# ClashLuke/LocAtE

Hardware: AMD Instinct MI355X
Metric: images/sec (G+D step) 64x64 bs=64 (higher is better)
Workload: dtype f32 (contractions fp32-faithful on the matrix cores: 2 x scaled fp16 operand pieces / 3 MFMAs per slice where the operand's largest magnitude comes with it, else 3 x bf16 pieces / 6 MFMAs; fp32 accumulate); 1 GPU; LocAtE G+D step, 64x64 RGB, batch 64 per GPU (the fp32 variant - the reference's own precision - of BASELINE.json configs[1]: 64x64 RGB bs 64), self/feature attention at 16x16 and 64x64, random-init weights; global_batch=64, image_size=64, parallelism=dp1, launch=hipGraph replay, G-step generator pass on a second stream

## Files before the change

locate_amd/csrc/conv.hip:

```cpp
#include "igemm.h"

template <int WGM, int WGN, int TM, int TN>
__global__ void __launch_bounds__(256) conv_igemm_kernel(const IgParams p) {
    constexpr int BK = IG_BK;
    constexpr int BM = WGM * TM * 32;
    constexpr int BN = WGN * TN * 32;
    constexpr int KPT = BK * BN / 256;
    constexpr int A_F4 = BK * BM / 4;
    constexpr int A_PT = (A_F4 + 255) / 256;
    static_assert(WGM * WGN == 4, "four waves");
    static_assert(BN % 64 == 0 && KPT == 8, "one 8-row group of the offset table per thread and step");
    static_assert(BK <= IG_TAIL, "panel tail shorter than the prefetch distance (one stage beyond the last)");

    __shared__ __attribute__((aligned(16))) float As[2][BK][BM];
    __shared__ __attribute__((aligned(16))) float Bs[2][BK][BN];

    int bx, by, bz;
    xcd_tile(bx, by, bz, p.tile_nphase);
    const int zphase = bz / p.ksplit, zsplit = bz - zphase * p.ksplit;
    const IgPhase& ph = p.ph[zphase];
    const int N = p.B * ph.QH * ph.QW;
    const int n0 = bx * BN;
    const int m0 = by * BM;
    if (n0 >= N) return;
// ... 91 lines not shown
        }
        __builtin_amdgcn_sched_barrier(0);
        store_tiles(buf ^ 1);
        __syncthreads();
    }

    igemm_epilogue<WGM, WGN, TM, TN>(p, ph, acc, col_scale, N, n0, m0, zsplit, wm, wn, lane, nullptr, p.ksplit > 1);
}

#define B6_BK 16

#define IG_FOUR_BLOCKS_TILES 3
#define IG_FOUR_BLOCKS_MIN 2
template <int WGM, int WGN, int TM, int TN, int NP, int NW = 4>
__global__ void __launch_bounds__(64 * NW, (NW == 8 ? 1 : (WGM * TM > 4 ? 2 : ((WGM * TM * TN <= IG_FOUR_BLOCKS_TILES && WGM * TM * TN >= IG_FOUR_BLOCKS_MIN && NP <= 2) ? 4 : 3)))) conv_igemm_bx6_kernel(const IgParams p) {
    constexpr int BK = 4 * NW, KB = BK / 8, KS = BK / 16, NT = 64 * NW;
    constexpr int BM = WGM * TM * 32;
    constexpr int BN = WGN * TN * 32;
    static_assert(NW == 4 || NW == 8, "four or eight waves");
    static_assert(WGM * WGN == NW, "wave grid");
    static_assert(BN == 128 && KB * BN == NT, "one gathered fragment (k-block) per thread and stage");
    static_assert(KB * BM <= 2 * NT, "at most two weight fragments per thread and stage");
    static_assert(B6_BK == 16, "the host's split-K accounting counts 16-deep steps");
    constexpr bool A2 = KB * BM > NT;
    static_assert(2 * BK <= IG_TAIL && (IG_TAIL % 8) == 0, "panel tail shorter than the prefetch distance");

    constexpr int A_U4 = 2 * NP * KB * BM, B_U4 = 2 * NP * KB * BN;
    constexpr int EPI_U4 = (NW * 32 * 33 + 8 + 3) / 4;
    constexpr int SMEM_U4 = A_U4 + B_U4 > EPI_U4 ? A_U4 + B_U4 : EPI_U4;
    __shared__ uint4 smem[SMEM_U4];
    uint4 (*As)[NP][KB][BM] = reinterpret_cast<uint4 (*)[NP][KB][BM]>(smem);
    uint4 (*Bs)[NP][KB][BN] = reinterpret_cast<uint4 (*)[NP][KB][BN]>(smem + A_U4);

    int bx, by, bz;
    xcd_tile(bx, by, bz, p.tile_nphase);
    const int zphase = bz / p.ksplit, zsplit = bz - zphase * p.ksplit;
    const IgPhase& ph = p.ph[zphase];
    const int N = p.B * ph.QH * ph.QW;
    const int n0 = bx * BN;
    const int m0 = by * BM;
    if (n0 >= N) return;

    const int tid = threadIdx.x, lane = tid & 63, wid = tid >> 6;
// ... 91 lines not shown
            Bs[buf][NP - 1][kgrp][ncol] = l;
        } else {
            bf16x8 h;
#pragma unroll
            for (int j = 0; j < 8; ++j) h[j] = (__bf16)breg[j];
            Bs[buf][0][kgrp][ncol] = *reinterpret_cast<uint4*>(&h);
        }
    };

    if (nsteps > 0) {
        issue_loads();
        store_tiles(0);
        issue_loads();
    }
    __syncthreads();
    const int lrow = lane >> 5, lcol = lane & 31;
    constexpr int PROD = NP == 3 ? 6 : (NP == 2 ? 3 : 1);
    constexpr int NMF = TM * TN * PROD, HALF = KS == 1 ? NMF / 2 : NMF;
    using frag_t = typename std::conditional<NP == 2, f16x8, bf16x8>::type;
    for (int s = 0; s < nsteps; ++s) {
        const int buf = s & 1;
        frag_t a[TM][NP], b[TN][NP];
        auto fragments = [&](int ksub) {
#pragma unroll
            for (int i = 0; i < TM; ++i)
#pragma unroll
                for (int q = 0; q < NP; ++q) a[i][q] = *reinterpret_cast<const frag_t*>(&As[buf][q][2 * ksub + lrow][(wm * TM + i) * 32 + lcol]);
#pragma unroll
            for (int j = 0; j < TN; ++j)
#pragma unroll
// ... 32 lines not shown
            mfmas(HALF, NMF);
        } else {
            fragments(1);
            mfmas(0, NMF);
        }
        if constexpr (NP >= 2) {
#pragma unroll
            for (int k = 0; k < (KS == 1 ? NMF - HALF : NMF); ++k) {
                __builtin_amdgcn_sched_group_barrier(0x008, 1, 0);
                __builtin_amdgcn_sched_group_barrier(0x020, 1, 0);
                __builtin_amdgcn_sched_group_barrier(0x002, 3, 0);
            }
        }
        __syncthreads();
    }
    if constexpr (NP == 2) {
#pragma unroll
        for (int i = 0; i < TM; ++i)
#pragma unroll
            for (int j = 0; j < TN; ++j)
#pragma unroll
                for (int r = 0; r < 16; ++r) acc[i][j][r] = (acc[i][j][r] * a_unscale) * b_unscale;
    }
    float* const stage = reinterpret_cast<float*>(smem) + wid * (32 * 33);
    bool combined = false;
    if (p.ksplit > 1 && p.combine) {
        constexpr int FR = TM * TN * 4;
        const int tile = (zphase * (int)gridDim.y + by) * (int)gridDim.x + bx;
        const int ntiles = p.nphase * (int)gridDim.y * (int)gridDim.x;
        const unsigned tile_bytes = FR * NT * 16;
        __amdgpu_buffer_rsrc_t srs = __builtin_amdgcn_make_buffer_rsrc(p.slab, 0, (int)((unsigned)p.ksplit * ntiles * tile_bytes), 0x00020000);
        const unsigned my = ((unsigned)(zsplit * ntiles + tile)) * tile_bytes + (unsigned)tid * 16u;
#pragma unroll
        for (int i = 0; i < TM; ++i)
#pragma unroll
            for (int j = 0; j < TN; ++j)
#pragma unroll
                for (int q = 0; q < 4; ++q) {
                    u32x4 v;
                    v[0] = __float_as_uint(acc[i][j][4 * q + 0]); v[1] = __float_as_uint(acc[i][j][4 * q + 1]);
                    v[2] = __float_as_uint(acc[i][j][4 * q + 2]); v[3] = __float_as_uint(acc[i][j][4 * q + 3]);
                    __builtin_amdgcn_raw_buffer_store_b128(v, srs, (int)(my + (unsigned)(((i * TN + j) * 4 + q) * NT * 16)), 0, 16);
                }
        asm volatile("s_waitcnt vmcnt(0)" ::: "memory");
        __syncthreads();
        unsigned* const flag = reinterpret_cast<unsigned*>(smem) + NW * 32 * 33 + 4;
        if (tid == 0) {
            const unsigned ticket = __hip_atomic_fetch_add(p.counters + tile, 1u, __ATOMIC_RELAXED, __HIP_MEMORY_SCOPE_AGENT);
            const bool last = ticket == (unsigned)(p.ksplit - 1);
            if (last) {
                __hip_atomic_store(p.counters + tile, 0u, __ATOMIC_RELAXED, __HIP_MEMORY_SCOPE_AGENT);
                __builtin_amdgcn_fence(__ATOMIC_ACQUIRE, "agent");
                asm volatile("s_waitcnt vmcnt(0)" ::: "memory");
            }
            *flag = last ? 1u : 0u;
        }
        __syncthreads();
        if (*flag == 0u) return;
        const unsigned t0 = (unsigned)tile * tile_bytes + (unsigned)tid * 16u;
        const unsigned zstride = (unsigned)ntiles * tile_bytes;
#pragma unroll
// ... 14 lines not shown
                        v[zz][f] = __builtin_amdgcn_raw_buffer_load_b128(srs, (int)(t0 + (unsigned)(z0 + zz) * zstride + (unsigned)((h0 + f) * NT * 16)), 0, 16);
#pragma unroll
                for (int zz = 0; zz < ZB; ++zz)
#pragma unroll
                    for (int f = 0; f < HB; ++f) {
                        const int g = h0 + f, i = g / (TN * 4), j = (g / 4) % TN, q = g % 4;
#pragma unroll
                        for (int e = 0; e < 4; ++e) acc[i][j][4 * q + e] += __uint_as_float(v[zz][f][e]);
                    }
            }
        }
        __syncthreads();
        combined = true;
    }
    igemm_epilogue<WGM, WGN, TM, TN>(p, ph, acc, col_scale, N, n0, m0, combined ? 0 : zsplit, wm, wn, lane, stage, p.ksplit > 1 && !combined);
}

__global__ void __launch_bounds__(256) igemm_slab_reduce_kernel(const float* __restrict__ slab, float* __restrict__ out,
                                                                const float* __restrict__ bias, const float* __restrict__ scale,
                                                                int scale_bg, int scale_stride, int B, int M, int plane,
                                                                long long out_bs, long long slab_stride, int ksplit,
                                                                float* __restrict__ act_out, long long act_bs,
                                                                const float* __restrict__ mul_pre, long long mul_bs,
                                                                unsigned* __restrict__ out_absmax) {
    const unsigned per_b = (unsigned)M * (unsigned)plane;
    const unsigned total = (unsigned)B * per_b;
    const unsigned stride = gridDim.x * blockDim.x;
    const DivU32 dpb(per_b), dpl((unsigned)plane);
    float am = 0.0f;
    for (unsigned i = blockIdx.x * blockDim.x + threadIdx.x; i < total; i += stride) {
// ... 280 lines not shown
                                                                              p.out_bs, p.slab_stride, p.ksplit, p.act_out, p.act_bs, p.mul_pre, p.mul_bs, p.out_absmax);
}

template <int NP>
static void launch_bx6(const IgParams& p, dim3 grid, int bm, bool w8, hipStream_t st) {
    if (w8) {
        if (bm == 128) conv_igemm_bx6_kernel<2, 4, 2, 1, NP, 8><<<grid, 512, 0, st>>>(p);
        else conv_igemm_bx6_kernel<2, 4, 1, 1, NP, 8><<<grid, 512, 0, st>>>(p);
        return;
    }
    with_tile<true>(bm, [&](auto t) { using T = decltype(t); conv_igemm_bx6_kernel<T::wgm, T::wgn, T::tm, T::tn, NP><<<grid, 256, 0, st>>>(p); });
}

static int launch_igemm(IgParams& p, int nmax, void* slab_ws, unsigned* counters, hipStream_t st, const char* who) {
    p.tile_nphase = (path_disabled("phasefast") || (long long)p.OH * p.OW < 1024) ? 1 : p.nphase;
    if (p.win) return launch_win_igemm(p, nmax, slab_ws, counters, st, who);
    if (skinny_ok(p)) {
        p.ksplit = 1;
        launch_skinny(p, st);
        LOCATE_LAUNCH_CHECK(who);
        return LOCATE_OK;
    }
    if (pointwise_ok(p)) {
        p.ksplit = 1;
        launch_pointwise(p, st);
        LOCATE_LAUNCH_CHECK(who);
        return LOCATE_OK;
    }
    const int bm = igemm_bm(p.M, nmax, p.nphase);
    const SplitPlan sp = igemm_split_plan(p, nmax, counters != nullptr);
    p.ksplit = sp.ksplit;
    p.combine = sp.combine;
    p.counters = counters;
    p.slab = static_cast<float*>(slab_ws);
    p.slab_stride = (long long)p.B * p.M * p.OH * p.OW;
    dim3 grid(sp.gx, sp.gy, p.nphase * p.ksplit);
    for (int i = 0; i < p.nphase; ++i)
        LOCATE_REQUIRE(round_up(p.M, bm) <= p.ph[i].ld, "%s: tile height %d does not divide the panel width %d", who, bm, p.ph[i].ld);
    if (p.precision == 3) {
        launch_fp8_igemm(p, grid, bm, st);
        LOCATE_LAUNCH_CHECK(who);
        if (p.ksplit > 1 && !p.combine) {
            LOCATE_REQUIRE(p.slab_stride < (1ll << 31), "%s: split-K output of %lld elements exceeds the 32-bit index range", who, p.slab_stride);
            launch_slab_reduce(p, st);
            LOCATE_LAUNCH_CHECK(who);
        }
        return LOCATE_OK;
    }
    const bool w8 = !path_disabled("w8") && !path_disabled("bx6") && (bm == 128 || bm == 64) &&
                    (long long)grid.x * grid.y * grid.z <= knob_int("LOCATE_W8_MAX", 320);
// ... 405 lines not shown
                     static_cast<unsigned*>(counters), precision, static_cast<const unsigned*>(x_absmax), as_stream(stream), "locate_conv_fwd",
                     static_cast<const LocateActEpilogue*>(act_epilogue));
}

LOCATE_API int locate_conv_dgrad(const int* geom, const float* gy, int64_t gy_bs, const float* panel, const float* scale,
                                 int scale_group_batch, int scale_stride, const float* bias, float* gx, int64_t gx_bs,
                                 void* workspace, void* counters, int precision, const void* gy_absmax, const void* act_epilogue,
                                 void* stream) {
    const ConvGeom g = make_geom(geom);
    if (int e = geom_check(g, "locate_conv_dgrad")) return e;
    LOCATE_REQUIRE(gy && panel && gx, "locate_conv_dgrad: null pointer");
    return run_igemm(g, 1, gy, gy_bs, panel, scale, scale_group_batch, scale_stride, bias, gx, gx_bs,
                     static_cast<float*>(workspace), static_cast<unsigned*>(counters), precision, static_cast<const unsigned*>(gy_absmax),
                     as_stream(stream), "locate_conv_dgrad", static_cast<const LocateActEpilogue*>(act_epilogue));
}
```

locate_amd/csrc/convfp8.hip:

```cpp
#include "igemm.h"

__device__ __forceinline__ uint4 quant_fp8x16(const float (&v)[16], float sc) {
    unsigned w[4];
#pragma unroll
    for (int q = 0; q < 4; ++q) {
        int t = 0;
        t = __builtin_amdgcn_cvt_pk_fp8_f32(v[4 * q + 0] * sc, v[4 * q + 1] * sc, t, false);
        t = __builtin_amdgcn_cvt_pk_fp8_f32(v[4 * q + 2] * sc, v[4 * q + 3] * sc, t, true);
        w[q] = (unsigned)t;
    }
    return make_uint4(w[0], w[1], w[2], w[3]);
}

template <int WGM, int WGN, int TM, int TN>
__global__ void __launch_bounds__(256, (WGM * TM > 4 ? 2 : 3)) conv_igemm_fp8_kernel(const IgParams p) {
    constexpr int BK = 32, KB = 2, NT = 256, NW = 4;
    constexpr int BM = WGM * TM * 32;
    constexpr int BN = WGN * TN * 32;
    static_assert(WGM * WGN == NW && BN == 128 && KB * BN == NT, "one gathered chunk (16 k) per thread and stage");
    static_assert(KB * BM <= 2 * NT, "at most two weight chunks per thread and stage");
    constexpr bool A2 = KB * BM > NT;
    static_assert(2 * BK <= IG_TAIL, "panel tail shorter than the prefetch distance");
    constexpr int A_U4 = 2 * KB * BM, B_U4 = 2 * KB * BN;
    constexpr int EPI_U4 = (NW * 32 * 33 + 8 + 3) / 4;
    constexpr int SMEM_U4 = A_U4 + B_U4 > EPI_U4 ? A_U4 + B_U4 : EPI_U4;
    __shared__ uint4 smem[SMEM_U4];
    uint4 (*As)[KB][BM] = reinterpret_cast<uint4 (*)[KB][BM]>(smem);
    uint4 (*Bs)[KB][BN] = reinterpret_cast<uint4 (*)[KB][BN]>(smem + A_U4);

    int bx, by, bz;
    xcd_tile(bx, by, bz, p.tile_nphase);
    const int zphase = bz / p.ksplit, zsplit = bz - zphase * p.ksplit;
    const IgPhase& ph = p.ph[zphase];
    const int N = p.B * ph.QH * ph.QW;
    const int n0 = bx * BN;
    const int m0 = by * BM;
    if (n0 >= N) return;

    const int tid = threadIdx.x, lane = tid & 63, wid = tid >> 6;
// ... 94 lines not shown
        mfmas(0, NMF / 2);
        __builtin_amdgcn_sched_barrier(0);
        store_tiles(buf ^ 1);
        __builtin_amdgcn_sched_barrier(0);
        issue_loads();
        mfmas(NMF / 2, NMF);
        __syncthreads();
    }
#pragma unroll
    for (int i = 0; i < TM; ++i)
#pragma unroll
        for (int j = 0; j < TN; ++j)
#pragma unroll
            for (int r = 0; r < 16; ++r) acc[i][j][r] = (acc[i][j][r] * a_unscale) * b_unscale;

    float* const stage = reinterpret_cast<float*>(smem) + wid * (32 * 33);
    bool combined = false;
    if (p.ksplit > 1 && p.combine) {
        constexpr int FR = TM * TN * 4;
        const int tile = (zphase * (int)gridDim.y + by) * (int)gridDim.x + bx;
        const int ntiles = p.nphase * (int)gridDim.y * (int)gridDim.x;
        const unsigned tile_bytes = FR * NT * 16;
        __amdgpu_buffer_rsrc_t srs = __builtin_amdgcn_make_buffer_rsrc(p.slab, 0, (int)((unsigned)p.ksplit * ntiles * tile_bytes), 0x00020000);
        const unsigned my = ((unsigned)(zsplit * ntiles + tile)) * tile_bytes + (unsigned)tid * 16u;
#pragma unroll
        for (int i = 0; i < TM; ++i)
#pragma unroll
            for (int j = 0; j < TN; ++j)
#pragma unroll
                for (int q = 0; q < 4; ++q) {
                    u32x4 v;
                    v[0] = __float_as_uint(acc[i][j][4 * q + 0]); v[1] = __float_as_uint(acc[i][j][4 * q + 1]);
                    v[2] = __float_as_uint(acc[i][j][4 * q + 2]); v[3] = __float_as_uint(acc[i][j][4 * q + 3]);
                    __builtin_amdgcn_raw_buffer_store_b128(v, srs, (int)(my + (unsigned)(((i * TN + j) * 4 + q) * NT * 16)), 0, 16);
                }
        asm volatile("s_waitcnt vmcnt(0)" ::: "memory");
        __syncthreads();
        unsigned* const flag = reinterpret_cast<unsigned*>(smem) + NW * 32 * 33 + 4;
        if (tid == 0) {
            const unsigned ticket = __hip_atomic_fetch_add(p.counters + tile, 1u, __ATOMIC_RELAXED, __HIP_MEMORY_SCOPE_AGENT);
            const bool last = ticket == (unsigned)(p.ksplit - 1);
            if (last) {
                __hip_atomic_store(p.counters + tile, 0u, __ATOMIC_RELAXED, __HIP_MEMORY_SCOPE_AGENT);
                __builtin_amdgcn_fence(__ATOMIC_ACQUIRE, "agent");
                asm volatile("s_waitcnt vmcnt(0)" ::: "memory");
            }
            *flag = last ? 1u : 0u;
        }
        __syncthreads();
        if (*flag == 0u) return;
        const unsigned t0 = (unsigned)tile * tile_bytes + (unsigned)tid * 16u;
        const unsigned zstride = (unsigned)ntiles * tile_bytes;
#pragma unroll
// ... 35 lines not shown
```

locate_amd/csrc/convwin.hip:

```cpp
#include "igemm.h"

typedef unsigned u32x2 __attribute__((ext_vector_type(2)));
typedef int i32x2 __attribute__((ext_vector_type(2)));
typedef int i32x4 __attribute__((ext_vector_type(4)));

template <int WGM, int WGN, int TM, int TN, int NP, int SL, int BPT>
__global__ void __launch_bounds__(256, 2) conv_win_kernel(const IgParams p) {
    constexpr int NT = 256, NW = 4, U = 2 * SL;
    constexpr int BM = WGM * TM * 32;
    constexpr int BN = WGN * TN * 32;
    static_assert(WGM * WGN == NW && (BN == 128 || BN == 256), "four waves on a 128- or 256-column tile");
    constexpr int A_CH = U * BM;
    constexpr int A_PT = (A_CH + NT - 1) / NT;
    constexpr int A_U4 = 2 * NP * A_CH;
    static_assert(2 * U <= WIN_TAIL_UNITS, "panel tail shorter than the prefetch distance");

    extern __shared__ uint4 smem[];

    int bx, by, bz;
    xcd_tile(bx, by, bz, p.tile_nphase);
    const int zphase = bz / p.ksplit, zsplit = bz - zphase * p.ksplit;
    const IgPhase& ph = p.ph[zphase];
    const int QHW = ph.QH * ph.QW;
    const int N = p.B * QHW;
// ... 29 lines not shown
        const bool ok = n < N;
        const int nn = ok ? n : n0;
        const int b = nn / QHW, q = nn - b * QHW;
        const int qy = q / ph.QW, qx = q - qy * ph.QW;
        const int iy0 = qy * p.istride, ix0 = qx * p.istride;
        unsigned inside = 0;
        for (int t = 0; t < T; ++t) {
            const int th = (t * ph.tw_magic) >> 16, tw = t - th * ph.TW;
            const bool in = (unsigned)(iy0 + ph.dy0 + ph.dys * th) < (unsigned)p.H && (unsigned)(ix0 + ph.dx0 + ph.dxs * tw) < (unsigned)p.W;
            inside |= (in ? 1u : 0u) << t;
        }
        outs[j] = ok ? (Tp == 1 ? 0u : ~inside) : ~0u;
        lbase[j] = ((b - b0) * WR + iy0 - iy_lo) * p.W + qx;
    }
    float col_scale[TN];
    igemm_col_scales<WGM, WGN, TM, TN>(p, ph, col_scale, N, n0, wn, lane);
    float b_scale = 1.0f, a_unscale = 1.0f, b_unscale = 1.0f;
    if constexpr (NP == 2) {
        const int kb_ = f16_scale_exp(absmax_read(p.b_absmax));
        const int ka_ = f16_scale_exp(__builtin_amdgcn_readfirstlane(*ph.a_absmax));
        b_scale = pow2f(kb_);
        unscale_pair(ka_, kb_, a_unscale, b_unscale);
    }

    f32x16 acc[TM][TN];
#pragma unroll
    for (int i = 0; i < TM; ++i)
#pragma unroll
        for (int j = 0; j < TN; ++j)
#pragma unroll
            for (int r = 0; r < 16; ++r) acc[i][j][r] = 0.0f;
// ... 245 lines not shown
                __builtin_amdgcn_sched_group_barrier(0x200, 1, 0);
                __builtin_amdgcn_sched_group_barrier(0x020, 1, 0);
            }
        }
        if (++g == NG) { g = 0; ++wrel; }
        __syncthreads();
    }
    if constexpr (NP == 2) {
#pragma unroll
        for (int i = 0; i < TM; ++i)
#pragma unroll
            for (int j = 0; j < TN; ++j)
#pragma unroll
                for (int r = 0; r < 16; ++r) acc[i][j][r] = (acc[i][j][r] * a_unscale) * b_unscale;
    }
    float* const stage = reinterpret_cast<float*>(smem) + wid * (32 * 33);
    bool combined = false;
    if (p.ksplit > 1 && p.combine) {
        constexpr int FR = TM * TN * 4;
        const int tile = (zphase * (int)gridDim.y + by) * (int)gridDim.x + bx;
        const int ntiles = p.nphase * (int)gridDim.y * (int)gridDim.x;
        const unsigned tile_bytes = FR * NT * 16;
        __amdgpu_buffer_rsrc_t srs = __builtin_amdgcn_make_buffer_rsrc(p.slab, 0, (int)((unsigned)p.ksplit * ntiles * tile_bytes), 0x00020000);
        const unsigned my = ((unsigned)(zsplit * ntiles + tile)) * tile_bytes + (unsigned)tid * 16u;
#pragma unroll
        for (int i = 0; i < TM; ++i)
#pragma unroll
            for (int j = 0; j < TN; ++j)
#pragma unroll
                for (int q = 0; q < 4; ++q) {
                    u32x4 v;
                    v[0] = __float_as_uint(acc[i][j][4 * q + 0]); v[1] = __float_as_uint(acc[i][j][4 * q + 1]);
                    v[2] = __float_as_uint(acc[i][j][4 * q + 2]); v[3] = __float_as_uint(acc[i][j][4 * q + 3]);
                    __builtin_amdgcn_raw_buffer_store_b128(v, srs, (int)(my + (unsigned)(((i * TN + j) * 4 + q) * NT * 16)), 0, 16);
                }
        asm volatile("s_waitcnt vmcnt(0)" ::: "memory");
        __syncthreads();
        unsigned* const flag = reinterpret_cast<unsigned*>(smem) + NW * 32 * 33 + 4;
        if (tid == 0) {
            const unsigned ticket = __hip_atomic_fetch_add(p.counters + tile, 1u, __ATOMIC_RELAXED, __HIP_MEMORY_SCOPE_AGENT);
            const bool last = ticket == (unsigned)(p.ksplit - 1);
            if (last) {
                __hip_atomic_store(p.counters + tile, 0u, __ATOMIC_RELAXED, __HIP_MEMORY_SCOPE_AGENT);
                __builtin_amdgcn_fence(__ATOMIC_ACQUIRE, "agent");
                asm volatile("s_waitcnt vmcnt(0)" ::: "memory");
            }
            *flag = last ? 1u : 0u;
        }
        __syncthreads();
        if (*flag == 0u) return;
        const unsigned t0 = (unsigned)tile * tile_bytes + (unsigned)tid * 16u;
        const unsigned zstride = (unsigned)ntiles * tile_bytes;
#pragma unroll
// ... 13 lines not shown
                    for (int f = 0; f < HB; ++f)
                        v[zz][f] = __builtin_amdgcn_raw_buffer_load_b128(srs, (int)(t0 + (unsigned)(z0 + zz) * zstride + (unsigned)((h0 + f) * NT * 16)), 0, 16);
#pragma unroll
                for (int zz = 0; zz < ZB; ++zz)
#pragma unroll
                    for (int f = 0; f < HB; ++f) {
                        const int gg = h0 + f, i = gg / (TN * 4), j = (gg / 4) % TN, q = gg % 4;
#pragma unroll
                        for (int e = 0; e < 4; ++e) acc[i][j][4 * q + e] += __uint_as_float(v[zz][f][e]);
                    }
            }
        }
        __syncthreads();
        combined = true;
    }
    igemm_epilogue<WGM, WGN, TM, TN>(p, ph, acc, col_scale, N, n0, m0, combined ? 0 : zsplit, wm, wn, lane, stage, p.ksplit > 1 && !combined);
}

struct WinSplit {
    int ksplit, combine, gx, gy;
    size_t slab_floats;
};

static int win_nwin(const IgParams& p) {
    const int C8G = (p.C + 7) / 8;
    return p.ph[0].win_Tp == 1 ? (C8G + p.win_U - 1) / p.win_U : C8G;
}

static WinSplit win_split_plan(const IgParams& p, int nmax, bool have_counters) {
    WinSplit sp;
    const int bm = p.win_bm;
// ... 72 lines not shown
    const int U = p.win_U, bm = p.win_bm;
    const bool single = p.ph[0].win_Tp == 1;
    for (int i = 0; i < p.nphase; ++i)
        LOCATE_REQUIRE(round_up(p.M, bm) <= p.ph[i].ld, "%s: tile height %d does not divide the panel width %d", who, bm, p.ph[i].ld);
    int bpt = 1;
    for (int i = 0; i < p.nphase; ++i) {
        const IgPhase& ph = p.ph[i];
        const long long items = (long long)(single ? U : 1) * (ph.win_NI * ph.win_WR * p.W / 2);
        const int need = (int)((items + 256ll * ph.win_NG - 1) / (256ll * ph.win_NG));
        if (need > bpt) bpt = need;
    }
    LOCATE_REQUIRE(bpt <= 2, "%s: window of %d items per thread", who, bpt);
    int ng_max = 1;
    for (int i = 0; i < p.nphase; ++i) ng_max = p.ph[i].win_NG > ng_max ? p.ph[i].win_NG : ng_max;
    size_t lds = ((size_t)2 * NP * U * bm + (size_t)2 * NP * (single ? U : 1) * p.win_slotsp) * 16 + (size_t)ng_max * bpt * 256 * 8;
    const size_t epi = (size_t)4 * 32 * 33 * 4 + 64;
    if (lds < epi) lds = epi;
    LOCATE_REQUIRE(lds <= 160 * 1024, "%s: window images of %zu bytes exceed the LDS", who, lds);
    dim3 grid(sp.gx, sp.gy, p.nphase * p.ksplit);
    if (NP == 2) win_launch_sl<2>(p, grid, lds, bpt, st);
    else if (NP == 3) win_launch_sl<3>(p, grid, lds, bpt, st);
    else win_launch_sl<1>(p, grid, lds, bpt, st);
    LOCATE_LAUNCH_CHECK(who);
    if (p.ksplit > 1 && !p.combine) {
        LOCATE_REQUIRE(p.slab_stride < (1ll << 31), "%s: split-K output of %lld elements exceeds the 32-bit index range", who, p.slab_stride);
        launch_slab_reduce(p, st);
        LOCATE_LAUNCH_CHECK(who);
    }
    return LOCATE_OK;
}
```

locate_amd/csrc/igemm.h:

```cpp
#pragma once
#include "common.h"
#include <cstdlib>
#include <cstring>
#include <stdlib.h>
#include <type_traits>

#ifdef LOCATE_DEBUG_KNOBS
static bool path_disabled(const char* name) {
    static const char* env = getenv("LOCATE_DISABLE");
    return env != nullptr && strstr(env, name) != nullptr;
}
static int knob_int(const char* name, int fallback) {
    const char* v = getenv(name);
    return v != nullptr ? atoi(v) : fallback;
}
#else
static constexpr bool path_disabled(const char*) { return false; }
static constexpr int knob_int(const char*, int fallback) { return fallback; }
#endif

typedef float f32x16 __attribute__((ext_vector_type(16)));

#define IG_BK 16
#define IG_KPAD 32
// ... 169 lines not shown
    h = *reinterpret_cast<unsigned*>(&hh);
    l = *reinterpret_cast<unsigned*>(&ll);
}

struct IgPhase {
    const float* wp;
    const int* koff;
    const unsigned char* ktap;
    const uint4* w3;
    const unsigned* a_absmax;
    long long w3_plane;
    int K, Kpad, ld, T;
    int dmin;
    int oy0, ox0, QH, QW;
    int TW, tw_magic;
    int dy0, dys, dx0, dxs;
    int win_Tp, win_NG, win_TR, win_NI, win_WR;
    unsigned win_wrw_mul;
    int win_wrw_s1, win_wrw_s2;
    int tapc[32] __attribute__((aligned(32)));
};

struct IgParams {
    const float* in;
    float* out;
    const float* bias;
    const float* scale;
    int scale_bg;
    int scale_stride;
    long long in_bs, out_bs;
// ... 5 lines not shown
    float* slab;
    long long slab_stride;
    int precision;
    const unsigned* b_absmax;
    float* act_out = nullptr;
    long long act_bs = 0;
    const float* lat = nullptr;
    long long lat_bs = 0;
    int lat_z = 0;
    const float* mul_pre = nullptr;
    long long mul_bs = 0;
    unsigned* out_absmax = nullptr;
    int combine;
    unsigned* counters;
    int tile_nphase;
    int win;
    int win_dbg;
    int win_U, win_slotsp, win_bm, win_bn;
    IgPhase ph[4];
};

template <int WGM, int WGN, int TM, int TN>
__device__ __forceinline__ void igemm_col_scales(const IgParams& p, const IgPhase& ph, float (&col_scale)[TN], int N, int n0,
                                                 int wn, int lane) {
    const int lcol = lane & 31;
#pragma unroll
    for (int j = 0; j < TN; ++j) {
        const int nj = n0 + (wn * TN + j) * 32 + lcol;
        const int nn = nj < N ? nj : 0;
        const int b = nn / (ph.QH * ph.QW);
        col_scale[j] = p.scale ? p.scale[(p.scale_bg ? b / p.scale_bg : 0) * p.scale_stride] : 1.0f;
    }
}

template <int WGM, int WGN, int TM, int TN>
__device__ __forceinline__ void igemm_epilogue(const IgParams& p, const IgPhase& ph, f32x16 (&acc)[TM][TN],
                                               const float (&col_scale)[TN], int N, int n0, int m0, int zsplit, int wm,
                                               int wn, int lane, float* stage, bool split) {
    const int lrow = lane >> 5, lcol = lane & 31;
    const long long plane = (long long)p.OH * p.OW;
    const int iplane = (int)plane;
    if (stage != nullptr && p.nphase == 1 && p.ostep == 1 && iplane <= 16 && (iplane & (iplane - 1)) == 0 &&
        ph.QH * ph.QW == iplane) {
        const int lp = __ffs(iplane) - 1;
        const bool fused_s = !split && (p.act_out != nullptr || p.mul_pre != nullptr);
        float am_s = 0.0f;
        float* out_base = split ? p.slab + (long long)zsplit * p.slab_stride : p.out;
        const long long obs = split ? (long long)p.M * plane : p.out_bs;
#pragma unroll
        for (int i = 0; i < TM; ++i) {
            const int mt0 = m0 + (wm * TM + i) * 32;
            float bias_v[16];
#pragma unroll
// ... 73 lines not shown
                }
                __builtin_amdgcn_fence(__ATOMIC_SEQ_CST, "wavefront");
            }
        }
        if (fused_s && p.out_absmax != nullptr) absmax_publish_wave(am_s, p.out_absmax);
        return;
    }
    const float* optr[TN];
    long long xoff[TN];
    const bool fused = !split && (p.act_out != nullptr || p.mul_pre != nullptr);
#pragma unroll
    for (int j = 0; j < TN; ++j) {
        const int nj = n0 + (wn * TN + j) * 32 + lcol;
        const int nn = nj < N ? nj : 0;
        const int qhw = ph.QH * ph.QW;
        const int b = nn / qhw, q = nn - b * qhw;
        const int qy = q / ph.QW, qx = q - qy * ph.QW;
        const long long pix = (long long)(ph.oy0 + qy * p.ostep) * p.OW + (ph.ox0 + qx * p.ostep);
        const float* o = split ? p.slab + (long long)zsplit * p.slab_stride + (long long)b * p.M * plane + pix
                               : p.out + (long long)b * p.out_bs + pix;
        optr[j] = nj < N ? o : nullptr;
        xoff[j] = (long long)b * ((p.mul_pre ? p.mul_bs : p.act_bs) - p.out_bs);
    }
    float am = 0.0f;
#pragma unroll
    for (int i = 0; i < TM; ++i) {
        float bias_v[16];
#pragma unroll
        for (int r = 0; r < 16; ++r) {
            const int m = m0 + (wm * TM + i) * 32 + (r & 3) + 8 * (r >> 2) + 4 * lrow;
            const bool use = p.bias != nullptr && !split && m < p.M;
            const float* bp = use ? p.bias + m : p.in;
// ... 30 lines not shown
            } else {
                float* ao = p.act_out + ((o - p.out) + xoff[j]);
#pragma unroll
                for (int r = 0; r < 16; ++r) {
                    const int m = m0 + (wm * TM + i) * 32 + (r & 3) + 8 * (r >> 2) + 4 * lrow;
                    const float v = fmaf(acc[i][j][r], col_scale[j], bias_v[r]);
                    const float a = roottanh_f(v);
                    if (m < p.M) { o[(long long)m * plane] = v; ao[(long long)m * plane] = a; am = fmaxf(am, fabsf(a)); }
                    if ((r & 7) == 7) __builtin_amdgcn_sched_barrier(0);
                }
            }
        }
    }
    if (fused && p.out_absmax != nullptr) absmax_publish_wave(am, p.out_absmax);
}

__device__ __forceinline__ void xcd_tile(int& bx, int& by, int& bz, int nphase = 1) {
    const int nx = gridDim.x, ny = gridDim.y;
    const int nwg = nx * ny * (int)gridDim.z;
    const int lin = blockIdx.x + nx * (blockIdx.y + ny * blockIdx.z);
    const int q = nwg >> 3, r = nwg & 7, xcd = lin & 7;
    int swz = (xcd < r ? xcd * (q + 1) : r * (q + 1) + (xcd - r) * q) + (lin >> 3);
    int phase = 0;
    if (nphase > 1) { phase = swz % nphase; swz /= nphase; }
    bx = swz % nx;
    const int t = swz / nx;
    by = t % ny;
    bz = t / ny;
    if (nphase > 1) bz += phase * ((int)gridDim.z / nphase);
}

struct GatherCol {
    __amdgpu_buffer_rsrc_t rsrc;
    unsigned lane_off;
    unsigned outside;
};

__device__ __forceinline__ GatherCol gather_setup(const IgParams& p, const IgPhase& ph, int n, int N) {
    GatherCol g;
    g.rsrc = __builtin_amdgcn_make_buffer_rsrc(const_cast<float*>(p.in + ph.dmin), 0, (int)(p.in_bytes - 4 * ph.dmin), 0x00020000);
    const bool n_ok = n < N;
    const int nn = n_ok ? n : 0;
    const int qhw = ph.QH * ph.QW;
    const int b = nn / qhw, q = nn - b * qhw;
    const int qy = q / ph.QW, qx = q - qy * ph.QW;
    const int iy0 = qy * p.istride, ix0 = qx * p.istride;
    g.lane_off = (unsigned)(4 * ((long long)b * p.in_bs + (long long)iy0 * p.W + ix0));
    unsigned inside = 0;
    if (n_ok) {
        for (int t = 0; t < ph.T; ++t) {
            const int th = (t * ph.tw_magic) >> 16, tw = t - th * ph.TW;
            const bool ok = (unsigned)(iy0 + ph.dy0 + ph.dys * th) < (unsigned)p.H &&
                            (unsigned)(ix0 + ph.dx0 + ph.dxs * tw) < (unsigned)p.W;
            inside |= (ok ? 1u : 0u) << t;
        }
    }
    g.outside = ~inside;
    return g;
}

__device__ __forceinline__ float gather_load(const GatherCol& g, int soff, unsigned tap) {
    const unsigned vo = ((g.outside << (31u - tap)) & 0x80000000u) | g.lane_off;
    return __builtin_bit_cast(float, __builtin_amdgcn_raw_buffer_load_b32(g.rsrc, (int)vo, soff, 0));
}

typedef int i32x8 __attribute__((ext_vector_type(8)));
typedef unsigned u32x4 __attribute__((ext_vector_type(4)));


__device__ __forceinline__ int fastdiv(int n, unsigned mul, int s1, int s2) {
    const unsigned t = __umulhi((unsigned)n, mul);
    return (int)((t + (((unsigned)n - t) >> s1)) >> s2);
}
static void fastdiv_make(unsigned d, unsigned* mul, int* s1, int* s2) {
    if (d <= 1) { *mul = 0; *s1 = 0; *s2 = 0; return; }
    int l = 0;
    while ((1ull << l) < d) ++l;
    *mul = (unsigned)(((1ull << 32) * ((1ull << l) - d)) / d + 1);
    *s1 = 1; *s2 = l - 1;
}

#define WIN_TAIL_UNITS 16

static inline int win_pick_bm(int M) { return (M >= 192 && M % 192 == 0) ? 192 : pick_bm(M); }
static inline int win_pick_bn(int bm) { return bm >= 128 ? 128 : 256; }
static inline int win_pick_sl(const int* X, int nx) {
    long long real = 0, padded = 0;
    for (int i = 0; i < nx; ++i) { real += X[i]; padded += (X[i] + 3) / 4 * 4; }
    return (padded - real) * 100 <= 15 * real ? 2 : 1;
}

static inline int win_pack_cs(int KK) { return KK <= 4 ? 64 : (KK <= 16 ? 32 : 16); }
static inline __host__ __device__ int win_pack_rg(int KK) { return KK == 1 ? 64 : 16; }
static inline size_t win_panel_floats(int urows, int ld, int fmt) { return PANEL_HDR + (size_t)(fmt ? 2 : 3) * urows * ld * 4; }

int launch_win_igemm(IgParams& p, int nmax, void* slab_ws, unsigned* counters, hipStream_t st, const char* who);
// ... 4 lines not shown
```

Measured before the change: 7263 images/sec.

## Add row-wise vectorized igemm epilogue stores and precomputed fast divisors

Adds a new epilogue path that stages each 32x32 accumulator tile in LDS with a padded pitch, then writes whole output rows as float4 stores, including fused activation, gradient-multiply and split-K slab variants. It is enabled when the layout is a single phase with stride-1 output and aligned planes. It also replaces integer divisions in the gather setup, column scales and epilogue with host-precomputed magic-multiply divisors. The aim is to replace scattered per-lane scalar stores and costly division sequences with coalesced wide stores, at the cost of extra LDS traffic and a larger epilogue staging area. Debug cycle-stamp instrumentation is added but compiled only under a debug macro.

New measurement: 7310 images/sec (median of 6 runs). About the same (+0.6%).

```diff
diff --git a/locate_amd/csrc/conv.hip b/locate_amd/csrc/conv.hip
--- a/locate_amd/csrc/conv.hip
+++ b/locate_amd/csrc/conv.hip
@@ -1,4 +1,29 @@
 #include "igemm.h"
+
+#ifdef LOCATE_DEBUG_KNOBS
+__device__ unsigned long long* igemm_dbg_cycles = nullptr;
+__device__ int igemm_dbg_blocks = 0;
+int igemm_dbg_last_rowst = -1;
+#define IG_DBG_BEGIN unsigned long long dbg_t0 = wall_clock64(), dbg_t1 = 0, dbg_t2 = 0
+#define IG_DBG_STAMP(t) t = wall_clock64()
+#define IG_DBG_END                                                                                                  \
+    do {                                                                                                            \
+        unsigned long long* const dbg_buf = igemm_dbg_cycles;                                                       \
+        if (dbg_buf != nullptr) {                                                                                   \
+            asm volatile("s_waitcnt vmcnt(0)" ::: "memory");                                                        \
+            const unsigned long long dbg_t3 = wall_clock64();                                                       \
+            const int dbg_lin = blockIdx.x + gridDim.x * (blockIdx.y + gridDim.y * blockIdx.z);                     \
+            if (threadIdx.x == 0 && dbg_lin < igemm_dbg_blocks) {                                                   \
+                dbg_buf[4 * dbg_lin + 0] = dbg_t0; dbg_buf[4 * dbg_lin + 1] = dbg_t1;                               \
+                dbg_buf[4 * dbg_lin + 2] = dbg_t2; dbg_buf[4 * dbg_lin + 3] = dbg_t3;                               \
+            }                                                                                                       \
+        }                                                                                                           \
+    } while (0)
+#else
+#define IG_DBG_BEGIN
+#define IG_DBG_STAMP(t)
+#define IG_DBG_END
+#endif
 
 template <int WGM, int WGN, int TM, int TN>
 __global__ void __launch_bounds__(256) conv_igemm_kernel(const IgParams p) {
@@ -129,6 +154,7 @@
 #define IG_FOUR_BLOCKS_MIN 2
 template <int WGM, int WGN, int TM, int TN, int NP, int NW = 4>
 __global__ void __launch_bounds__(64 * NW, (NW == 8 ? 1 : (WGM * TM > 4 ? 2 : ((WGM * TM * TN <= IG_FOUR_BLOCKS_TILES && WGM * TM * TN >= IG_FOUR_BLOCKS_MIN && NP <= 2) ? 4 : 3)))) conv_igemm_bx6_kernel(const IgParams p) {
+    IG_DBG_BEGIN;
     constexpr int BK = 4 * NW, KB = BK / 8, KS = BK / 16, NT = 64 * NW;
     constexpr int BM = WGM * TM * 32;
     constexpr int BN = WGN * TN * 32;
@@ -141,7 +167,7 @@
     static_assert(2 * BK <= IG_TAIL && (IG_TAIL % 8) == 0, "panel tail shorter than the prefetch distance");
 
     constexpr int A_U4 = 2 * NP * KB * BM, B_U4 = 2 * NP * KB * BN;
-    constexpr int EPI_U4 = (NW * 32 * 33 + 8 + 3) / 4;
+    constexpr int EPI_U4 = (NW * IG_PATCH + 8 + 3) / 4;
     constexpr int SMEM_U4 = A_U4 + B_U4 > EPI_U4 ? A_U4 + B_U4 : EPI_U4;
     __shared__ uint4 smem[SMEM_U4];
     uint4 (*As)[NP][KB][BM] = reinterpret_cast<uint4 (*)[NP][KB][BM]>(smem);
@@ -263,6 +289,7 @@
         issue_loads();
     }
     __syncthreads();
+    IG_DBG_STAMP(dbg_t1);
     const int lrow = lane >> 5, lcol = lane & 31;
     constexpr int PROD = NP == 3 ? 6 : (NP == 2 ? 3 : 1);
     constexpr int NMF = TM * TN * PROD, HALF = KS == 1 ? NMF / 2 : NMF;
@@ -325,6 +352,7 @@
         }
         __syncthreads();
     }
+    IG_DBG_STAMP(dbg_t2);
     if constexpr (NP == 2) {
 #pragma unroll
         for (int i = 0; i < TM; ++i)
@@ -333,7 +361,7 @@
 #pragma unroll
                 for (int r = 0; r < 16; ++r) acc[i][j][r] = (acc[i][j][r] * a_unscale) * b_unscale;
     }
-    float* const stage = reinterpret_cast<float*>(smem) + wid * (32 * 33);
+    float* const stage = reinterpret_cast<float*>(smem) + wid * IG_PATCH;
     bool combined = false;
     if (p.ksplit > 1 && p.combine) {
         constexpr int FR = TM * TN * 4;
@@ -355,7 +383,7 @@
                 }
         asm volatile("s_waitcnt vmcnt(0)" ::: "memory");
         __syncthreads();
-        unsigned* const flag = reinterpret_cast<unsigned*>(smem) + NW * 32 * 33 + 4;
+        unsigned* const flag = reinterpret_cast<unsigned*>(smem) + NW * IG_PATCH + 4;
         if (tid == 0) {
             const unsigned ticket = __hip_atomic_fetch_add(p.counters + tile, 1u, __ATOMIC_RELAXED, __HIP_MEMORY_SCOPE_AGENT);
             const bool last = ticket == (unsigned)(p.ksplit - 1);
@@ -400,6 +428,7 @@
         combined = true;
     }
     igemm_epilogue<WGM, WGN, TM, TN>(p, ph, acc, col_scale, N, n0, m0, combined ? 0 : zsplit, wm, wn, lane, stage, p.ksplit > 1 && !combined);
+    IG_DBG_END;
 }
 
 __global__ void __launch_bounds__(256) igemm_slab_reduce_kernel(const float* __restrict__ slab, float* __restrict__ out,
@@ -710,6 +739,11 @@
 
 static int launch_igemm(IgParams& p, int nmax, void* slab_ws, unsigned* counters, hipStream_t st, const char* who) {
     p.tile_nphase = (path_disabled("phasefast") || (long long)p.OH * p.OW < 1024) ? 1 : p.nphase;
+    igemm_fill_divisors(p);
+    p.rowst = 0;
+#ifdef LOCATE_DEBUG_KNOBS
+    igemm_dbg_last_rowst = 0;
+#endif
     if (p.win) return launch_win_igemm(p, nmax, slab_ws, counters, st, who);
     if (skinny_ok(p)) {
         p.ksplit = 1;
@@ -730,6 +764,10 @@
     p.counters = counters;
     p.slab = static_cast<float*>(slab_ws);
     p.slab_stride = (long long)p.B * p.M * p.OH * p.OW;
+    p.rowst = igemm_row_stores_ok(p) ? 1 : 0;
+#ifdef LOCATE_DEBUG_KNOBS
+    igemm_dbg_last_rowst = p.rowst;
+#endif
     dim3 grid(sp.gx, sp.gy, p.nphase * p.ksplit);
     for (int i = 0; i < p.nphase; ++i)
         LOCATE_REQUIRE(round_up(p.M, bm) <= p.ph[i].ld, "%s: tile height %d does not divide the panel width %d", who, bm, p.ph[i].ld);
@@ -1165,3 +1203,12 @@
                      static_cast<float*>(workspace), static_cast<unsigned*>(counters), precision, static_cast<const unsigned*>(gy_absmax),
                      as_stream(stream), "locate_conv_dgrad", static_cast<const LocateActEpilogue*>(act_epilogue));
 }
+
+#ifdef LOCATE_DEBUG_KNOBS
+LOCATE_API int locate_debug_igemm_cycles(void* cycles, int blocks) {
+    unsigned long long* buf = static_cast<unsigned long long*>(cycles);
+    if (hipMemcpyToSymbol(HIP_SYMBOL(igemm_dbg_blocks), &blocks, sizeof(blocks)) != hipSuccess) return 1;
+    return hipMemcpyToSymbol(HIP_SYMBOL(igemm_dbg_cycles), &buf, sizeof(buf)) != hipSuccess;
+}
+LOCATE_API int locate_debug_last_row_stores(void) { return igemm_dbg_last_rowst; }
+#endif
diff --git a/locate_amd/csrc/convfp8.hip b/locate_amd/csrc/convfp8.hip
--- a/locate_amd/csrc/convfp8.hip
+++ b/locate_amd/csrc/convfp8.hip
@@ -22,7 +22,7 @@
     constexpr bool A2 = KB * BM > NT;
     static_assert(2 * BK <= IG_TAIL, "panel tail shorter than the prefetch distance");
     constexpr int A_U4 = 2 * KB * BM, B_U4 = 2 * KB * BN;
-    constexpr int EPI_U4 = (NW * 32 * 33 + 8 + 3) / 4;
+    constexpr int EPI_U4 = (NW * IG_PATCH + 8 + 3) / 4;
     constexpr int SMEM_U4 = A_U4 + B_U4 > EPI_U4 ? A_U4 + B_U4 : EPI_U4;
     __shared__ uint4 smem[SMEM_U4];
     uint4 (*As)[KB][BM] = reinterpret_cast<uint4 (*)[KB][BM]>(smem);
@@ -147,7 +147,7 @@
 #pragma unroll
             for (int r = 0; r < 16; ++r) acc[i][j][r] = (acc[i][j][r] * a_unscale) * b_unscale;
 
-    float* const stage = reinterpret_cast<float*>(smem) + wid * (32 * 33);
+    float* const stage = reinterpret_cast<float*>(smem) + wid * IG_PATCH;
     bool combined = false;
     if (p.ksplit > 1 && p.combine) {
         constexpr int FR = TM * TN * 4;
@@ -169,7 +169,7 @@
                 }
         asm volatile("s_waitcnt vmcnt(0)" ::: "memory");
         __syncthreads();
-        unsigned* const flag = reinterpret_cast<unsigned*>(smem) + NW * 32 * 33 + 4;
+        unsigned* const flag = reinterpret_cast<unsigned*>(smem) + NW * IG_PATCH + 4;
         if (tid == 0) {
             const unsigned ticket = __hip_atomic_fetch_add(p.counters + tile, 1u, __ATOMIC_RELAXED, __HIP_MEMORY_SCOPE_AGENT);
             const bool last = ticket == (unsigned)(p.ksplit - 1);
diff --git a/locate_amd/csrc/convwin.hip b/locate_amd/csrc/convwin.hip
--- a/locate_amd/csrc/convwin.hip
+++ b/locate_amd/csrc/convwin.hip
@@ -67,7 +67,7 @@
         lbase[j] = ((b - b0) * WR + iy0 - iy_lo) * p.W + qx;
     }
     float col_scale[TN];
-    igemm_col_scales<WGM, WGN, TM, TN>(p, ph, col_scale, N, n0, wn, lane);
+    igemm_col_scales<WGM, WGN, TM, TN, false>(p, ph, col_scale, N, n0, wn, lane);
     float b_scale = 1.0f, a_unscale = 1.0f, b_unscale = 1.0f;
     if constexpr (NP == 2) {
         const int kb_ = f16_scale_exp(absmax_read(p.b_absmax));
@@ -343,7 +343,7 @@
 #pragma unroll
                 for (int r = 0; r < 16; ++r) acc[i][j][r] = (acc[i][j][r] * a_unscale) * b_unscale;
     }
-    float* const stage = reinterpret_cast<float*>(smem) + wid * (32 * 33);
+    float* const stage = reinterpret_cast<float*>(smem) + wid * IG_PATCH;
     bool combined = false;
     if (p.ksplit > 1 && p.combine) {
         constexpr int FR = TM * TN * 4;
@@ -365,7 +365,7 @@
                 }
         asm volatile("s_waitcnt vmcnt(0)" ::: "memory");
         __syncthreads();
-        unsigned* const flag = reinterpret_cast<unsigned*>(smem) + NW * 32 * 33 + 4;
+        unsigned* const flag = reinterpret_cast<unsigned*>(smem) + NW * IG_PATCH + 4;
         if (tid == 0) {
             const unsigned ticket = __hip_atomic_fetch_add(p.counters + tile, 1u, __ATOMIC_RELAXED, __HIP_MEMORY_SCOPE_AGENT);
             const bool last = ticket == (unsigned)(p.ksplit - 1);
@@ -409,7 +409,7 @@
         __syncthreads();
         combined = true;
     }
-    igemm_epilogue<WGM, WGN, TM, TN>(p, ph, acc, col_scale, N, n0, m0, combined ? 0 : zsplit, wm, wn, lane, stage, p.ksplit > 1 && !combined);
+    igemm_epilogue<WGM, WGN, TM, TN, false>(p, ph, acc, col_scale, N, n0, m0, combined ? 0 : zsplit, wm, wn, lane, stage, p.ksplit > 1 && !combined);
 }
 
 struct WinSplit {
@@ -512,7 +512,7 @@
     int ng_max = 1;
     for (int i = 0; i < p.nphase; ++i) ng_max = p.ph[i].win_NG > ng_max ? p.ph[i].win_NG : ng_max;
     size_t lds = ((size_t)2 * NP * U * bm + (size_t)2 * NP * (single ? U : 1) * p.win_slotsp) * 16 + (size_t)ng_max * bpt * 256 * 8;
-    const size_t epi = (size_t)4 * 32 * 33 * 4 + 64;
+    const size_t epi = (size_t)4 * IG_PATCH * 4 + 64;
     if (lds < epi) lds = epi;
     LOCATE_REQUIRE(lds <= 160 * 1024, "%s: window images of %zu bytes exceed the LDS", who, lds);
     dim3 grid(sp.gx, sp.gy, p.nphase * p.ksplit);
diff --git a/locate_amd/csrc/igemm.h b/locate_amd/csrc/igemm.h
--- a/locate_amd/csrc/igemm.h
+++ b/locate_amd/csrc/igemm.h
@@ -207,6 +207,8 @@
     int dmin;
     int oy0, ox0, QH, QW;
     int TW, tw_magic;
+    unsigned qhw_mul, qw_mul;
+    int qhw_s1, qhw_s2, qw_s1, qw_s2;
     int dy0, dys, dx0, dxs;
     int win_Tp, win_NG, win_TR, win_NI, win_WR;
     unsigned win_wrw_mul;
@@ -242,13 +244,57 @@
     int combine;
     unsigned* counters;
     int tile_nphase;
+    int rowst;
+    unsigned plane_mul;
+    int plane_s1, plane_s2;
+    unsigned sbg_mul;
+    int sbg_s1, sbg_s2;
     int win;
     int win_dbg;
     int win_U, win_slotsp, win_bm, win_bn;
     IgPhase ph[4];
 };
 
-template <int WGM, int WGN, int TM, int TN>
+__device__ __forceinline__ int fastdiv(int n, unsigned mul, int s1, int s2) {
+    const unsigned t = __umulhi((unsigned)n, mul);
+    return (int)((t + (((unsigned)n - t) >> s1)) >> s2);
+}
+static void fastdiv_make(unsigned d, unsigned* mul, int* s1, int* s2) {
+    if (d <= 1) { *mul = 0; *s1 = 0; *s2 = 0; return; }
+    int l = 0;
+    while ((1ull << l) < d) ++l;
+    *mul = (unsigned)(((1ull << 32) * ((1ull << l) - d)) / d + 1);
+    *s1 = 1; *s2 = l - 1;
+}
+
+static inline void igemm_fill_divisors(IgParams& p) {
+    for (int i = 0; i < p.nphase; ++i) {
+        IgPhase& ph = p.ph[i];
+        fastdiv_make((unsigned)(ph.QH * ph.QW), &ph.qhw_mul, &ph.qhw_s1, &ph.qhw_s2);
+        fastdiv_make((unsigned)ph.QW, &ph.qw_mul, &ph.qw_s1, &ph.qw_s2);
+    }
+    fastdiv_make((unsigned)(p.OH * p.OW), &p.plane_mul, &p.plane_s1, &p.plane_s2);
+    fastdiv_make((unsigned)(p.scale_bg > 0 ? p.scale_bg : 1), &p.sbg_mul, &p.sbg_s1, &p.sbg_s2);
+}
+
+#define IG_PATCH_PITCH 36
+#define IG_PATCH (32 * IG_PATCH_PITCH)
+
+static inline bool igemm_row_stores_ok(const IgParams& p) {
+    if (path_disabled("rowstores")) return false;
+    const long long plane = (long long)p.OH * p.OW;
+    if (p.nphase != 1 || p.ostep != 1 || plane % 32 != 0) return false;
+    const IgPhase& ph = p.ph[0];
+    if (ph.oy0 != 0 || ph.ox0 != 0 || (long long)ph.QH * ph.QW != plane) return false;
+    const long long per = (long long)p.M * plane;
+    auto ok = [&](const void* base, long long bs) {
+        return (reinterpret_cast<uintptr_t>(base) & 15) == 0 && bs >= per && (bs & 3) == 0 && (long long)(p.B - 1) * bs + per < (1ll << 31);
+    };
+    if (p.ksplit > 1 && !p.combine) return ok(p.slab, per);
+    return ok(p.out, p.out_bs) && (!p.act_out || ok(p.act_out, p.act_bs)) && (!p.mul_pre || ok(p.mul_pre, p.mul_bs));
+}
+
+template <int WGM, int WGN, int TM, int TN, bool LEAN = true>
 __device__ __forceinline__ void igemm_col_scales(const IgParams& p, const IgPhase& ph, float (&col_scale)[TN], int N, int n0,
                                                  int wn, int lane) {
     const int lcol = lane & 31;
@@ -256,15 +302,118 @@
     for (int j = 0; j < TN; ++j) {
         const int nj = n0 + (wn * TN + j) * 32 + lcol;
         const int nn = nj < N ? nj : 0;
-        const int b = nn / (ph.QH * ph.QW);
-        col_scale[j] = p.scale ? p.scale[(p.scale_bg ? b / p.scale_bg : 0) * p.scale_stride] : 1.0f;
-    }
-}
-
-template <int WGM, int WGN, int TM, int TN>
+        if constexpr (LEAN) {
+            const int b = fastdiv(nn, ph.qhw_mul, ph.qhw_s1, ph.qhw_s2);
+            col_scale[j] = p.scale ? p.scale[(p.scale_bg ? fastdiv(b, p.sbg_mul, p.sbg_s1, p.sbg_s2) : 0) * p.scale_stride] : 1.0f;
+        } else {
+            const int b = nn / (ph.QH * ph.QW);
+            col_scale[j] = p.scale ? p.scale[(p.scale_bg ? b / p.scale_bg : 0) * p.scale_stride] : 1.0f;
+        }
+    }
+}
+
+enum { EPI_PLAIN = 0, EPI_SLAB = 1, EPI_ACT = 2, EPI_MUL = 3 };
+
+__device__ __forceinline__ int epi_row(int r, int lrow) { return (r & 3) + 8 * (r >> 2) + 4 * lrow; }
+
+__device__ __forceinline__ void epi_bias(const IgParams& p, int mt0, int lrow, bool split, float (&bias_v)[16]) {
+#pragma unroll
+    for (int r = 0; r < 16; ++r) {
+        const int m = mt0 + epi_row(r, lrow);
+        const bool use = p.bias != nullptr && !split && m < p.M;
+        const float* bp = use ? p.bias + m : p.in;
+        bias_v[r] = use ? *bp : 0.0f;
+    }
+}
+
+template <int KIND>
+__device__ __forceinline__ float epi_value(float acc, float scale, float bias) {
+    return KIND == EPI_SLAB ? acc : fmaf(acc, scale, bias);
+}
+
+template <int KIND, int WGM, int WGN, int TM, int TN>
+__device__ __forceinline__ void epi_rows(const IgParams& p, f32x16 (&acc)[TM][TN], const float (&col_scale)[TN], int N, int n0,
+                                         int m0, int zsplit, int wm, int wn, int lane, float* stage) {
+    const int lrow = lane >> 5, lcol = lane & 31;
+    const unsigned plane = (unsigned)(p.OH * p.OW);
+    float* const out_base = KIND == EPI_SLAB ? p.slab + (long long)zsplit * p.slab_stride : p.out;
+    const unsigned obs = KIND == EPI_SLAB ? (unsigned)p.M * plane : (unsigned)p.out_bs;
+    const unsigned xbs = KIND == EPI_MUL ? (unsigned)p.mul_bs : (unsigned)p.act_bs;
+    const int rl = lane >> 3, c4 = (lane & 7) * 4;
+    const unsigned lane_off = (unsigned)rl * plane + (unsigned)c4;
+    const float* const rd = stage + rl * IG_PATCH_PITCH + c4;
+    float am = 0.0f;
+#pragma unroll
+    for (int i = 0; i < TM; ++i) {
+        const int mt0 = m0 + (wm * TM + i) * 32;
+        float bias_v[16];
+        epi_bias(p, mt0, lrow, KIND == EPI_SLAB, bias_v);
+#pragma unroll
+        for (int j = 0; j < TN; ++j) {
+            const int nt0 = n0 + (wn * TN + j) * 32;
+            if (nt0 >= N) continue;
+#pragma unroll
+            for (int r = 0; r < 16; ++r)
+                stage[epi_row(r, lrow) * IG_PATCH_PITCH + lcol] = epi_value<KIND>(acc[i][j][r], col_scale[j], bias_v[r]);
+            __builtin_amdgcn_fence(__ATOMIC_SEQ_CST, "wavefront");
+            const unsigned b = (unsigned)fastdiv(nt0, p.plane_mul, p.plane_s1, p.plane_s2);
+            const unsigned rel = (unsigned)mt0 * plane + ((unsigned)nt0 - b * plane);
+            float* const o = out_base + (b * obs + rel) + lane_off;
+            float4 v[4];
+#pragma unroll
+            for (int e = 0; e < 4; ++e) v[e] = *reinterpret_cast<const float4*>(rd + e * 8 * IG_PATCH_PITCH);
+            if constexpr (KIND == EPI_PLAIN || KIND == EPI_SLAB) {
+#pragma unroll
+                for (int e = 0; e < 4; ++e)
+                    if (mt0 + e * 8 + rl < p.M) *reinterpret_cast<float4*>(o + (unsigned)(e * 8) * plane) = v[e];
+            } else if constexpr (KIND == EPI_MUL) {
+                const float* const pre = p.mul_pre + (b * xbs + rel) + lane_off;
+                float4 z[4];
+#pragma unroll
+                for (int e = 0; e < 4; ++e) {
+                    z[e] = make_float4(0.0f, 0.0f, 0.0f, 0.0f);
+                    if (mt0 + e * 8 + rl < p.M) z[e] = *reinterpret_cast<const float4*>(pre + (unsigned)(e * 8) * plane);
+                }
+#pragma unroll
+                for (int e = 0; e < 4; ++e) {
+                    if (mt0 + e * 8 + rl < p.M) {
+                        float4 g;
+                        g.x = roottanh_grad_f(z[e].x, v[e].x); g.y = roottanh_grad_f(z[e].y, v[e].y);
+                        g.z = roottanh_grad_f(z[e].z, v[e].z); g.w = roottanh_grad_f(z[e].w, v[e].w);
+                        am = fmaxf(fmaxf(fmaxf(am, fabsf(g.x)), fabsf(g.y)), fmaxf(fabsf(g.z), fabsf(g.w)));
+                        *reinterpret_cast<float4*>(o + (unsigned)(e * 8) * plane) = g;
+                    }
+                }
+            } else {
+                float* const ao = p.act_out + (b * xbs + rel) + lane_off;
+#pragma unroll
+                for (int e = 0; e < 4; ++e) {
+                    if (mt0 + e * 8 + rl < p.M) {
+                        float4 a;
+                        a.x = roottanh_f(v[e].x); a.y = roottanh_f(v[e].y); a.z = roottanh_f(v[e].z); a.w = roottanh_f(v[e].w);
+                        am = fmaxf(fmaxf(fmaxf(am, fabsf(a.x)), fabsf(a.y)), fmaxf(fabsf(a.z), fabsf(a.w)));
+                        *reinterpret_cast<float4*>(o + (unsigned)(e * 8) * plane) = v[e];
+                        *reinterpret_cast<float4*>(ao + (unsigned)(e * 8) * plane) = a;
+                    }
+                }
+            }
+            __builtin_amdgcn_fence(__ATOMIC_SEQ_CST, "wavefront");
+        }
+    }
+    if ((KIND == EPI_ACT || KIND == EPI_MUL) && p.out_absmax != nullptr) absmax_publish_wave(am, p.out_absmax);
+}
+
+template <int WGM, int WGN, int TM, int TN, bool LEAN = true>
 __device__ __forceinline__ void igemm_epilogue(const IgParams& p, const IgPhase& ph, f32x16 (&acc)[TM][TN],
                                                const float (&col_scale)[TN], int N, int n0, int m0, int zsplit, int wm,
                                                int wn, int lane, float* stage, bool split) {
+    if (LEAN && stage != nullptr && p.rowst) {
+        if (split) epi_rows<EPI_SLAB, WGM, WGN, TM, TN>(p, acc, col_scale, N, n0, m0, zsplit, wm, wn, lane, stage);
+        else if (p.mul_pre != nullptr) epi_rows<EPI_MUL, WGM, WGN, TM, TN>(p, acc, col_scale, N, n0, m0, zsplit, wm, wn, lane, stage);
+        else if (p.act_out != nullptr) epi_rows<EPI_ACT, WGM, WGN, TM, TN>(p, acc, col_scale, N, n0, m0, zsplit, wm, wn, lane, stage);
+        else epi_rows<EPI_PLAIN, WGM, WGN, TM, TN>(p, acc, col_scale, N, n0, m0, zsplit, wm, wn, lane, stage);
+        return;
+    }
     const int lrow = lane >> 5, lcol = lane & 31;
     const long long plane = (long long)p.OH * p.OW;
     const int iplane = (int)plane;
@@ -368,8 +517,8 @@
         const int nj = n0 + (wn * TN + j) * 32 + lcol;
         const int nn = nj < N ? nj : 0;
         const int qhw = ph.QH * ph.QW;
-        const int b = nn / qhw, q = nn - b * qhw;
-        const int qy = q / ph.QW, qx = q - qy * ph.QW;
+        const int b = LEAN ? fastdiv(nn, ph.qhw_mul, ph.qhw_s1, ph.qhw_s2) : nn / qhw, q = nn - b * qhw;
+        const int qy = LEAN ? fastdiv(q, ph.qw_mul, ph.qw_s1, ph.qw_s2) : q / ph.QW, qx = q - qy * ph.QW;
         const long long pix = (long long)(ph.oy0 + qy * p.ostep) * p.OW + (ph.ox0 + qx * p.ostep);
         const float* o = split ? p.slab + (long long)zsplit * p.slab_stride + (long long)b * p.M * plane + pix
                                : p.out + (long long)b * p.out_bs + pix;
@@ -430,6 +579,7 @@
     }
     if (fused && p.out_absmax != nullptr) absmax_publish_wave(am, p.out_absmax);
 }
+
 
 __device__ __forceinline__ void xcd_tile(int& bx, int& by, int& bz, int nphase = 1) {
     const int nx = gridDim.x, ny = gridDim.y;
@@ -457,9 +607,8 @@
     g.rsrc = __builtin_amdgcn_make_buffer_rsrc(const_cast<float*>(p.in + ph.dmin), 0, (int)(p.in_bytes - 4 * ph.dmin), 0x00020000);
     const bool n_ok = n < N;
     const int nn = n_ok ? n : 0;
-    const int qhw = ph.QH * ph.QW;
-    const int b = nn / qhw, q = nn - b * qhw;
-    const int qy = q / ph.QW, qx = q - qy * ph.QW;
+    const int b = fastdiv(nn, ph.qhw_mul, ph.qhw_s1, ph.qhw_s2), q = nn - b * (ph.QH * ph.QW);
+    const int qy = fastdiv(q, ph.qw_mul, ph.qw_s1, ph.qw_s2), qx = q - qy * ph.QW;
     const int iy0 = qy * p.istride, ix0 = qx * p.istride;
     g.lane_off = (unsigned)(4 * ((long long)b * p.in_bs + (long long)iy0 * p.W + ix0));
     unsigned inside = 0;
@@ -484,18 +633,6 @@
 typedef unsigned u32x4 __attribute__((ext_vector_type(4)));
 
 
-__device__ __forceinline__ int fastdiv(int n, unsigned mul, int s1, int s2) {
-    const unsigned t = __umulhi((unsigned)n, mul);
-    return (int)((t + (((unsigned)n - t) >> s1)) >> s2);
-}
-static void fastdiv_make(unsigned d, unsigned* mul, int* s1, int* s2) {
-    if (d <= 1) { *mul = 0; *s1 = 0; *s2 = 0; return; }
-    int l = 0;
-    while ((1ull << l) < d) ++l;
-    *mul = (unsigned)(((1ull << 32) * ((1ull << l) - d)) / d + 1);
-    *s1 = 1; *s2 = l - 1;
-}
-
 #define WIN_TAIL_UNITS 16
 
 static inline int win_pick_bm(int M) { return (M >= 192 && M % 192 == 0) ? 192 : pick_bm(M); }
```
